# mengcaopku/DCNet

Measured on AMD Instinct MI355X. Metric: clips/sec (T=8, 416x416, bs8) fwd+bwd, higher is better.
Workload: dtype f32; 1 GPU; T=8 416x416 bs8/GPU L=20 fp32, 64 img/GPU/step as pairs, fwd+5 losses+bwd+RMSprop; arith=f16x2-split MFMA, fp32 accumulate, parallelism=dp1, ranks_seen=1, reducer=none, step=hipGraph replay (fwd+losses+bwd+RMSprop), sampler=mt

## Files before the change

dcnet_amd/csrc/conv3x.hip:

```cpp
#include "igemm.h"
#include "prof.h"
#include <type_traits>

namespace {

typedef _Float16 f16x8_t __attribute__((ext_vector_type(8)));
typedef _Float16 f16x4_t __attribute__((ext_vector_type(4)));
constexpr unsigned OOBX = 0x80000000u;

constexpr int XBM = 256, XBN = 128, XNT = 512, XWM = 4;
constexpr int XPB = XBN * 32;
constexpr int XPB1 = XPB + 64;
constexpr int XSLOT = 2 * XPB + 128;
constexpr int XSTAGE = 6 * XSLOT;
constexpr int XA_LD = 4;
#ifndef C3X_ABL
#define C3X_ABL 0
#endif
constexpr int XSMAX = 466;
constexpr int XPA = (XSMAX + 2) * 32;

__device__ __forceinline__ f32x4 ldx16(__amdgpu_buffer_rsrc_t r, unsigned voff, unsigned soff) {
  return __builtin_bit_cast(f32x4, __builtin_amdgcn_raw_buffer_load_b128(r, voff, soff, 0));
}
__device__ __forceinline__ __amdgpu_buffer_rsrc_t rsrcx(const float* base, long long bytes) {
  const unsigned n = bytes > 0x7FFFFFF0LL ? 0x7FFFFFF0u : (bytes < 0 ? 0u : (unsigned)bytes);
  return __builtin_amdgcn_make_buffer_rsrc((void*)base, 0, n, 0x00020000);
}
__device__ __forceinline__ float pow2_scalex(unsigned amax_bits) {
  const int be = (int)((amax_bits >> 23) & 0xFF);
  if (be == 0 || be == 255) return 1.f;
  int e = 14 - (be - 126);
  e = e > 100 ? 100 : (e < -100 ? -100 : e);
  return __uint_as_float((unsigned)(e + 127) << 23);
}

typedef __attribute__((address_space(3))) void lds_voidx;
template <bool DMA>
__global__ __launch_bounds__(XNT, 2) void conv3x_kernel(const IgemmParams p, const int S, const int gran) {
  extern __shared__ __attribute__((aligned(16))) unsigned char smemx[];
  constexpr int PA = XPA;
  unsigned char* const Abase = smemx;
  unsigned char* const Bbase = smemx + 4 * PA;

  const int tid = threadIdx.x, lane = tid & 63, wave = tid >> 6;
  const int wm = wave >> 1, wn = wave & 1;
  const int c16 = lane & 15, g = lane >> 4, tsel = g >> 1, half = g & 1;
  const int gn = (p.Co + XBN - 1) / XBN;
  const int lin = xcd_remap(blockIdx.x, gridDim.x);
  const int bm = lin / gn, bn = lin - bm * gn;
  const int W = p.Wi, H = p.Hi, M = p.M;
  const int m0 = bm * XBM;
  const float sa = pow2_scalex(amax_read(p.amax_a)), sb = p.b_scale[0];

  const int lin0 = m0 - W - 1;
  const int base_px = lin0 > 0 ? lin0 : 0;
  const float* a_base = p.in + (long long)base_px * p.ldi;
  const __amdgpu_buffer_rsrc_t a_rs = rsrcx(a_base, ((long long)(M - base_px - 1) * p.ldi + p.Ci) * 4);
  const __amdgpu_buffer_rsrc_t b_rs = rsrcx(p.wt, (long long)p.Co * p.ldw * 4);

  const int pos0 = tid >> 2, q0 = tid & 3;
  const unsigned a_off0 = (unsigned)((lin0 + pos0 - base_px) * p.ldi * 4 + q0 * 16);
  const int a_st0 = pos0 * 32 + q0 * 8;
  const unsigned a_pstride = (unsigned)(128 * p.ldi * 4);
  bool a_ok[XA_LD], a_in[XA_LD];
#pragma unroll
  for (int j = 0; j < XA_LD; ++j) {
    const int pos = pos0 + 128 * j, px = lin0 + pos;
    a_in[j] = pos < S;
    a_ok[j] = pos < S && px >= 0 && px < M;
  }
  auto a_off = [&](const int j) {
    unsigned o = a_off0;
    asm volatile("" : "+v"(o));
    return a_ok[j] ? o + (unsigned)j * a_pstride : OOBX;
  };
  auto a_st = [&](const int j) {
    int o = a_st0;
    asm volatile("" : "+v"(o));
    return a_in[j] ? o + j * 4096 : (XSMAX + 1) * 32 + q0 * 8;
  };
  unsigned b_off; int b_st;
  if constexpr (DMA) {
    const int plane = wave & 1, rho = 32 * (wave >> 1) + (lane >> 1), kh = lane & 1;
    const int filt = (rho & ~63) + 4 * (rho & 15) + ((rho & 63) >> 4);
    const int co = bn * XBN + filt;
    b_off = co < p.Co ? (unsigned)(co * p.ldw * 4 + (2 * kh + plane) * 16) : OOBX;
    b_st = __builtin_amdgcn_readfirstlane(plane * XPB1 + (wave >> 1) * 1024);
  } else {
    const int rho = tid >> 2, chunk = tid & 3;
    const int filt = (rho & ~63) + 4 * (rho & 15) + ((rho & 63) >> 4);
    const int co = bn * XBN + filt;
    b_off = co < p.Co ? (unsigned)(co * p.ldw * 4 + chunk * 16) : OOBX;
    b_st = (chunk & 1) * XPB1 + rho * 32 + (chunk >> 1) * 16;
  }
  unsigned msk[4];
#pragma unroll
  for (int i = 0; i < 4; ++i) {
    const int m = m0 + wm * 64 + i * 16 + c16;
    unsigned v = 0;
    if (m < M) {
      const int rem = m % (H * W), y = rem / W, x = rem - y * W;
      for (int t = 0; t < 9; ++t)
        if ((unsigned)(y + p.tap_dy[t]) < (unsigned)H && (unsigned)(x + p.tap_dx[t]) < (unsigned)W) v |= 1u << t;
    }
    msk[i] = v;
  }
  const int a_lane0 = (wm * 64 + c16) * 32 + half * 16;
  const int b_lane0 = (wn * 64 + c16) * 32 + half * 16 + tsel * 3 * XSLOT;

  const int nch = p.Ci >> 4;
  const int nper = nch >> 1;
  const int nsi = 3 * nper;

  f32x4 a_reg[XA_LD], b_reg[6];
  const unsigned lds0 = (unsigned)(uintptr_t)(lds_voidx*)smemx;
  auto store_a_piece = [&](const int buf_off, int j) {
    const f32x4 t = a_reg[j] * sa;
    const f16x4_t h = {(_Float16)t[0], (_Float16)t[1], (_Float16)t[2], (_Float16)t[3]};
    const f16x4_t l = {(_Float16)(t[0] - (float)h[0]), (_Float16)(t[1] - (float)h[1]), (_Float16)(t[2] - (float)h[2]),
                       (_Float16)(t[3] - (float)h[3])};
    if constexpr (DMA) {
      const unsigned addr = lds0 + (unsigned)(buf_off + a_st(j));
      asm volatile("ds_write_b64 %0, %1\n\tds_write_b64 %0, %2 offset:%3"
                   :: "v"(addr), "v"(__builtin_bit_cast(unsigned long long, h)), "v"(__builtin_bit_cast(unsigned long long, l)), "n"(XPA));
    } else {
      unsigned char* abuf = Abase + buf_off;
      *reinterpret_cast<uint2*>(abuf + a_st(j)) = __builtin_bit_cast(uint2, h);
      *reinterpret_cast<uint2*>(abuf + PA + a_st(j)) = __builtin_bit_cast(uint2, l);
    }
  };

  f32x4 acc[4][4];
#pragma unroll
  for (int i = 0; i < 4; ++i)
#pragma unroll
    for (int j = 0; j < 4; ++j) acc[i][j] = f32x4{0.f, 0.f, 0.f, 0.f};

  if (tid < 8) {
    const f32x4 z = {0.f, 0.f, 0.f, 0.f};
    *reinterpret_cast<f32x4*>(Abase + (tid >> 1) * PA + XSMAX * 32 + (tid & 1) * 16) = z;
  }
#pragma unroll
  for (int j = 0; j < XA_LD; ++j) a_reg[j] = ldx16(a_rs, a_off(j), 0u);
  auto dma = [&](const int stage_off, const int slot, const bool live, const unsigned soff) {
    __builtin_amdgcn_raw_ptr_buffer_load_lds(b_rs, (lds_voidx*)(Bbase + stage_off + slot * XSLOT + b_st), 16, (int)(live ? b_off : OOBX),
                                             (int)(live ? soff : 0u), 0, 0);
  };
  if constexpr (DMA) {
#pragma unroll
    for (int q = 0; q < 6; ++q) {
      const int G = q / 3, j = q - 3 * G;
      dma(0, q, true, (unsigned)p.tap_w[3 * G + j] * 4u);
    }
#pragma unroll
    for (int q = 0; q < 2; ++q)
      dma(XSTAGE, q, true, (unsigned)p.tap_w[6 + q] * 4u);
#pragma unroll
    for (int j = 0; j < XA_LD; ++j) store_a_piece(0, j);
#pragma unroll
    for (int j = 0; j < XA_LD; ++j) a_reg[j] = ldx16(a_rs, a_off(j), 64u);
    asm volatile("s_waitcnt vmcnt(0)" ::: "memory");
  } else {
#pragma unroll
    for (int q = 0; q < 6; ++q) {
      const int G = q / 3, j = q - 3 * G;
      b_reg[q] = ldx16(b_rs, b_off, (unsigned)p.tap_w[3 * G + j] * 4u);
    }
#pragma unroll
    for (int j = 0; j < XA_LD; ++j) store_a_piece(0, j);
#pragma unroll
    for (int j = 0; j < XA_LD; ++j) a_reg[j] = ldx16(a_rs, a_off(j), 64u);
#pragma unroll
    for (int q = 0; q < 6; ++q) *reinterpret_cast<f32x4*>(Bbase + q * XSLOT + b_st) = b_reg[q];
#pragma unroll
    for (int q = 0; q < 6; ++q) {
      const int G = q < 3 ? 2 : 0, cc = q < 3 ? 0 : 1, j = q % 3;
      b_reg[q] = ldx16(b_rs, b_off, (unsigned)(p.tap_w[3 * G + j] + cc * 16) * 4u);
    }
  }
  __syncthreads();

  f16x8_t Al[4], Ah[4], Bh[4], Bl[4];
  int ad[4];
  auto a_addr = [&](const int T, const int J) {
    const int Ga = T == 0 ? 0 : (T == 1 ? 2 : 1), Gb = T == 0 ? 1 : (T == 1 ? 0 : 2);
    const int ta = 3 * Ga + J, tb = 3 * Gb + J;
    const int sha = (p.tap_dy[ta] + 1) * W + p.tap_dx[ta] + 1, shb = (p.tap_dy[tb] + 1) * W + p.tap_dx[tb] + 1;
    int ts = tsel;
    asm volatile("" : "+v"(ts));
    const int sh = ts ? shb : sha;
    const int tl = ts ? tb : ta;
    const int bo = T == 0 ? 0 : (T == 2 ? 2 * PA : ts * (2 * PA));
    const int base = bo + a_lane0 + sh * 32;
    const int z = bo + XSMAX * 32;
#pragma unroll
    for (int i = 0; i < 4; ++i) ad[i] = ((msk[i] >> tl) & 1) ? base + i * 512 : z;
  };
  auto read_Al = [&]() {
#pragma unroll
    for (int i = 0; i < 4; ++i) Al[i] = *reinterpret_cast<const f16x8_t*>(Abase + PA + ad[i]);
  };
  auto read_Ah = [&]() {
#pragma unroll
    for (int i = 0; i < 4; ++i) Ah[i] = *reinterpret_cast<const f16x8_t*>(Abase + ad[i]);
  };
  int st_cur = 0;
  auto read_B = [&](f16x8_t (&B)[4], const int stage_off, const int J, const int plane) {
    const unsigned char* bb = Bbase + stage_off + b_lane0;
#pragma unroll
    for (int jn = 0; jn < 4; ++jn) B[jn] = *reinterpret_cast<const f16x8_t*>(bb + J * XSLOT + plane * XPB1 + jn * 512);
  };
  auto mm = [&](const f16x8_t (&A)[4], const f16x8_t (&B)[4]) {
#pragma unroll
    for (int i = 0; i < 4; ++i)
#pragma unroll
      for (int jn = 0; jn < 4; ++jn) acc[i][jn] = __builtin_amdgcn_mfma_f32_16x16x32_f16(A[i], B[jn], acc[i][jn], 0, 0, 0);
  };

  auto body = [&](auto T_, const int u) {
    constexpr int T = decltype(T_)::value;
    constexpr int TN = (T + 1) % 3;
    const int k = 3 * u + T, c0 = 2 * u;
    const bool in_b = k + 2 < nsi;
    const int st_nxt = XSTAGE - st_cur;
    unsigned char* const bw = Bbase + st_nxt + b_st;
    auto side = [&](const int gi) {
      if constexpr (DMA) {
        if (gi < 4 && !(C3X_ABL & 1)) {
          const int sl = gi + 2, second = sl >= 3, j = sl - 3 * second;
          const int G = T == 0 ? (second ? 0 : 2) : (T == 1 ? (second ? 2 : 1) : (second ? 1 : 0));
          const int dc = T == 0 ? (second ? 1 : 0) : (T == 1 ? 1 : 2);
          dma(st_nxt, sl, k + 1 < nsi, (unsigned)(p.tap_w[3 * G + j] + (c0 + dc) * 16) * 4u);
        }
        if (gi >= 7 && !(C3X_ABL & 1)) {
          const int sl = gi - 7;
          const int G = T == 0 ? 1 : (T == 1 ? 0 : 2), dc = T == 0 ? 1 : 2;
          dma(st_cur, sl, in_b, (unsigned)(p.tap_w[3 * G + sl] + (c0 + dc) * 16) * 4u);
        }
      } else {
      if (gi < 6 && !(C3X_ABL & 4)) *reinterpret_cast<f32x4*>(bw + gi * XSLOT) = b_reg[gi];
      if (gi >= 3 && !(C3X_ABL & 1)) {
        const int q = gi - 3, second = q >= 3, j = q - 3 * second;
        const int G = T == 0 ? (second ? 2 : 1) : (T == 1 ? (second ? 1 : 0) : (second ? 0 : 2));
        const int dc = T == 0 ? 1 : (T == 1 ? 2 : (second ? 3 : 2));
        const unsigned soff = (unsigned)(p.tap_w[3 * G + j] + (c0 + dc) * 16) * 4u;
        b_reg[q] = ldx16(b_rs, in_b ? b_off : OOBX, in_b ? soff : 0u);
      }
      }
      if (T == 0 && gi >= 2 && gi < 2 + XA_LD && !(C3X_ABL & 4)) store_a_piece(2 * PA, gi - 2);
      if (T == 1 && gi < XA_LD && !(C3X_ABL & 2)) {
        const bool in_a = c0 + 2 < nch;
        a_reg[gi] = ldx16(a_rs, in_a ? a_off(gi) : OOBX, in_a ? (unsigned)(c0 + 2) * 64u : 0u);
      }
      if (T == 2 && gi < XA_LD && !(C3X_ABL & 4)) store_a_piece(0, gi);
      if (T == 2 && gi >= 4 && gi < 4 + XA_LD && !(C3X_ABL & 2)) {
        const bool in_a = c0 + 3 < nch;
        a_reg[gi - 4] = ldx16(a_rs, in_a ? a_off(gi - 4) : OOBX, in_a ? (unsigned)(c0 + 3) * 64u : 0u);
      }
    };
#pragma unroll
    for (int j = 0; j < 3; ++j) {
      read_Ah();
      read_B(Bl, st_cur, j, 1);
      __builtin_amdgcn_sched_barrier(0);
      mm(Al, Bh);
      side(3 * j);
      __builtin_amdgcn_sched_barrier(0);
      if (j == 2 && !(C3X_ABL & 8)) {
        if constexpr (DMA) {
          if (T == 2 && !(C3X_ABL & 2)) asm volatile("s_waitcnt vmcnt(3) lgkmcnt(0)\n\ts_barrier" ::: "memory");
          else asm volatile("s_waitcnt vmcnt(0) lgkmcnt(0)\n\ts_barrier" ::: "memory");
        } else {
          __syncthreads();
        }
      }
      if (j < 2) a_addr(T, j + 1); else a_addr(TN, 0);
      read_Al();
      __builtin_amdgcn_sched_barrier(0);
      mm(Ah, Bh);
      side(3 * j + 1);
      __builtin_amdgcn_sched_barrier(0);
      if (j < 2) read_B(Bh, st_cur, j + 1, 0); else read_B(Bh, st_nxt, 0, 0);
      __builtin_amdgcn_sched_barrier(0);
      mm(Ah, Bl);
      side(3 * j + 2);
      __builtin_amdgcn_sched_barrier(0);
    }
    st_cur = st_nxt;
  };
  a_addr(0, 0);
  read_Al();
  read_B(Bh, 0, 0, 0);
  {
    using I0 = std::integral_constant<int, 0>; using I1 = std::integral_constant<int, 1>; using I2 = std::integral_constant<int, 2>;
    for (int u = 0; u < nper; ++u) { body(I0{}, u); body(I1{}, u); body(I2{}, u); }
  }
  if constexpr (DMA) asm volatile("s_waitcnt vmcnt(0)" ::: "memory");
  __syncthreads();

  const float dq = 1.f / (sa * sb);
#pragma unroll
  for (int i = 0; i < 4; ++i)
#pragma unroll
    for (int jn = 0; jn < 4; ++jn) acc[i][jn] *= dq;
  const int co0 = bn * XBN + wn * 64 + 4 * c16;
  const bool co_ok = co0 < p.Co;
  const int mrow0 = m0 + wm * 64 + 4 * g;
  float* __restrict__ gout = p.out;
  if (p.accumulate && co_ok) {
#pragma unroll
    for (int i = 0; i < 4; ++i)
#pragma unroll
      for (int r = 0; r < 4; ++r) {
        const int m = mrow0 + 16 * i + r;
        if (m >= M) continue;
        const f32x4 o = *reinterpret_cast<const f32x4*>(gout + (size_t)m * p.ldo + co0);
#pragma unroll
        for (int jn = 0; jn < 4; ++jn) acc[i][jn][r] += o[jn];
      }
  }
  if (p.stats) {
    float* red = reinterpret_cast<float*>(smemx);
    float s[4] = {0.f, 0.f, 0.f, 0.f}, ss[4] = {0.f, 0.f, 0.f, 0.f};
    if (p.bt_y && co_ok) {
      const f32x4 mu = *reinterpret_cast<const f32x4*>(p.bt_mean + co0), is = *reinterpret_cast<const f32x4*>(p.bt_invstd + co0);
      f32x4 ga = {1.f, 1.f, 1.f, 1.f}, be = {0.f, 0.f, 0.f, 0.f};
      if (p.bt_gamma) ga = *reinterpret_cast<const f32x4*>(p.bt_gamma + co0);
      if (p.bt_beta) be = *reinterpret_cast<const f32x4*>(p.bt_beta + co0);
      const float* yb = p.bt_y + co0;
#pragma unroll
      for (int i = 0; i < 4; ++i) {
        f32x4 yv[4];
#pragma unroll
        for (int r = 0; r < 4; ++r) {
          const int m = mrow0 + 16 * i + r;
          yv[r] = *reinterpret_cast<const f32x4*>(yb + (size_t)(m < M ? m : M - 1) * p.Co);
        }
#pragma unroll
        for (int r = 0; r < 4; ++r) {
          const int m = mrow0 + 16 * i + r;
#pragma unroll
          for (int jn = 0; jn < 4; ++jn) {
            const float xh = (yv[r][jn] - mu[jn]) * is[jn];
            float gq = acc[i][jn][r];
            if (p.bt_act == DCN_ACT_LEAKY) gq = (ga[jn] * xh + be[jn] <= 0.f) ? gq * p.bt_slope : gq;
            gq = m < M ? gq : 0.f;
            s[jn] += gq; ss[jn] += gq * xh;
          }
        }
      }
    } else if (!p.bt_y) {
#pragma unroll
      for (int i = 0; i < 4; ++i)
#pragma unroll
        for (int r = 0; r < 4; ++r)
#pragma unroll
          for (int jn = 0; jn < 4; ++jn) { const float v = acc[i][jn][r]; s[jn] += v; ss[jn] = __builtin_fmaf(v, v, ss[jn]); }
    }
#pragma unroll
    for (int jn = 0; jn < 4; ++jn) {
      s[jn] += __shfl_xor(s[jn], 16); ss[jn] += __shfl_xor(ss[jn], 16);
      s[jn] += __shfl_xor(s[jn], 32); ss[jn] += __shfl_xor(ss[jn], 32);
    }
    if (g == 0) {
      const int col = wn * 64 + 4 * c16;
      *reinterpret_cast<f32x4*>(red + (0 * XWM + wm) * XBN + col) = f32x4{s[0], s[1], s[2], s[3]};
      *reinterpret_cast<f32x4*>(red + (1 * XWM + wm) * XBN + col) = f32x4{ss[0], ss[1], ss[2], ss[3]};
    }
    __syncthreads();
    const int groups = XBM / gran, spg = XWM / groups;
    const int rows_total = (M + gran - 1) / gran;
    for (int idx = tid; idx < 2 * XBN * groups; idx += XNT) {
      const int gq = idx / (2 * XBN), rest = idx - gq * 2 * XBN;
      const int which = rest / XBN, col = rest - which * XBN;
      float t = 0.f;
      for (int w = 0; w < spg; ++w) t += red[(which * XWM + gq * spg + w) * XBN + col];
      const int co = bn * XBN + col, srow = bm * groups + gq;
      if (co < p.Co && srow < rows_total) p.stats[((size_t)srow * 2 + which) * p.Co + co] = t;
    }
  }
  float vmax = 0.f;
  if (co_ok) {
    f32x4 sc = {1.f, 1.f, 1.f, 1.f}, sh = {0.f, 0.f, 0.f, 0.f};
    if (p.scale) sc = *reinterpret_cast<const f32x4*>(p.scale + co0);
    if (p.shift) sh = *reinterpret_cast<const f32x4*>(p.shift + co0);
#pragma unroll
    for (int i = 0; i < 4; ++i)
#pragma unroll
      for (int r = 0; r < 4; ++r) {
        const int m = mrow0 + 16 * i + r;
        if (m >= M) continue;
        f32x4 v;
#pragma unroll
        for (int jn = 0; jn < 4; ++jn) {
          float t = acc[i][jn][r] * sc[jn] + sh[jn];
          if (p.act == DCN_ACT_LEAKY) t = t > 0.f ? t : t * p.slope;
          v[jn] = t;
        }
        if (p.residual) v += *reinterpret_cast<const f32x4*>(p.residual + (size_t)m * p.ldr + co0);
        *reinterpret_cast<f32x4*>(gout + (size_t)m * p.ldo + co0) = v;
#pragma unroll
        for (int jn = 0; jn < 4; ++jn) vmax = fmaxf(vmax, fabsf(v[jn]));
      }
  }
  if (p.amax_out) {
    vmax = wave_max(vmax);
    if (lane == 0) amax_update(p.amax_out, vmax, blockIdx.x * 8 + wave);
  }
}

}

bool conv3x_takes(const IgemmParams& p, int gran) {
  if (p.wt16 || (gran != 128 && gran != 256)) return false;
  if (p.Co % 4 != 0 || p.ldo % 4 != 0 || (p.residual && p.ldr % 4 != 0)) return false;
  auto al16 = [](const void* q) { return (reinterpret_cast<uintptr_t>(q) & 15) == 0; };
  if (!al16(p.out) || !al16(p.residual) || !al16(p.bt_y) || !al16(p.scale) || !al16(p.shift) || !al16(p.bt_mean) || !al16(p.bt_invstd) ||
      !al16(p.bt_gamma) || !al16(p.bt_beta)) return false;
  const int S = XBM + 2 * p.Wi + 2;
  if (S > XSMAX) return false;
  return (long long)S * p.ldi * 4 < 0x7FFFFFF0LL && (long long)p.Co * p.ldw * 4 < 0x7FFFFFF0LL;
}

int conv3x_launch(const IgemmParams& p, int gran, hipStream_t stream) {
  const int S = XBM + 2 * p.Wi + 2;
  const size_t lds = (size_t)4 * XPA + (size_t)2 * XSTAGE;
  static_assert((size_t)4 * XPA + (size_t)2 * XSTAGE <= 160 * 1024, "LDS");
  static DcnPerDeviceFlag attr_once;
  if (attr_once.first()) {
    (void)hipFuncSetAttribute(reinterpret_cast<const void*>(&conv3x_kernel<true>), hipFuncAttributeMaxDynamicSharedMemorySize, 160 * 1024);
  }
  const int gm = cdiv(p.M, XBM), gn = cdiv(p.Co, XBN);
  const double k_alg = 9.0 * p.Ci;
  const double alg_bytes = 4.0 * ((double)p.N * p.Hi * p.Wi * p.Ci + (double)p.Co * k_alg + (double)p.M * p.Co * epilogue_reads(p));
  const int pid = prof_begin(51, 2.0 * (double)p.M * p.Co * k_alg, stream, alg_bytes);
  hipLaunchKernelGGL(conv3x_kernel<true>, dim3(gm * gn), dim3(XNT), lds, stream, p, S, gran);
  prof_end(pid, stream);
  DCN_CHECK_LAUNCH("conv3x");
  return DCN_OK;
}
```

Measured before the change: 90.50 clips/s.

## Make conv3x persistent with next-tile prefetch overlapping the epilogue

```diff
diff --git a/dcnet_amd/csrc/conv3x.hip b/dcnet_amd/csrc/conv3x.hip
--- a/dcnet_amd/csrc/conv3x.hip
+++ b/dcnet_amd/csrc/conv3x.hip
@@ -19,6 +19,10 @@
 #endif
 constexpr int XSMAX = 466;
 constexpr int XPA = (XSMAX + 2) * 32;
+constexpr int XRED = 4 * XPA + 2 * XSTAGE;
+#ifndef C3X_WALK
+#define C3X_WALK 1
+#endif
 
 __device__ __forceinline__ f32x4 ldx16(__amdgpu_buffer_rsrc_t r, unsigned voff, unsigned soff) {
   return __builtin_bit_cast(f32x4, __builtin_amdgcn_raw_buffer_load_b128(r, voff, soff, 0));
@@ -47,29 +51,21 @@
   const int wm = wave >> 1, wn = wave & 1;
   const int c16 = lane & 15, g = lane >> 4, tsel = g >> 1, half = g & 1;
   const int gn = (p.Co + XBN - 1) / XBN;
-  const int lin = xcd_remap(blockIdx.x, gridDim.x);
-  const int bm = lin / gn, bn = lin - bm * gn;
   const int W = p.Wi, H = p.Hi, M = p.M;
-  const int m0 = bm * XBM;
+  const int tiles = ((M + XBM - 1) / XBM) * gn;
   const float sa = pow2_scalex(amax_read(p.amax_a)), sb = p.b_scale[0];
-
-  const int lin0 = m0 - W - 1;
-  const int base_px = lin0 > 0 ? lin0 : 0;
-  const float* a_base = p.in + (long long)base_px * p.ldi;
-  const __amdgpu_buffer_rsrc_t a_rs = rsrcx(a_base, ((long long)(M - base_px - 1) * p.ldi + p.Ci) * 4);
   const __amdgpu_buffer_rsrc_t b_rs = rsrcx(p.wt, (long long)p.Co * p.ldw * 4);
 
+  int bm, bn, m0;
+  __amdgpu_buffer_rsrc_t a_rs;
+
   const int pos0 = tid >> 2, q0 = tid & 3;
-  const unsigned a_off0 = (unsigned)((lin0 + pos0 - base_px) * p.ldi * 4 + q0 * 16);
+  unsigned a_off0;
   const int a_st0 = pos0 * 32 + q0 * 8;
   const unsigned a_pstride = (unsigned)(128 * p.ldi * 4);
   bool a_ok[XA_LD], a_in[XA_LD];
 #pragma unroll
-  for (int j = 0; j < XA_LD; ++j) {
-    const int pos = pos0 + 128 * j, px = lin0 + pos;
-    a_in[j] = pos < S;
-    a_ok[j] = pos < S && px >= 0 && px < M;
-  }
+  for (int j = 0; j < XA_LD; ++j) a_in[j] = pos0 + 128 * j < S;
   auto a_off = [&](const int j) {
     unsigned o = a_off0;
     asm volatile("" : "+v"(o));
@@ -80,32 +76,45 @@
     asm volatile("" : "+v"(o));
     return a_in[j] ? o + j * 4096 : (XSMAX + 1) * 32 + q0 * 8;
   };
-  unsigned b_off; int b_st;
+  unsigned b_off; int b_st, b_filt, b_chunk;
   if constexpr (DMA) {
     const int plane = wave & 1, rho = 32 * (wave >> 1) + (lane >> 1), kh = lane & 1;
-    const int filt = (rho & ~63) + 4 * (rho & 15) + ((rho & 63) >> 4);
-    const int co = bn * XBN + filt;
-    b_off = co < p.Co ? (unsigned)(co * p.ldw * 4 + (2 * kh + plane) * 16) : OOBX;
+    b_filt = (rho & ~63) + 4 * (rho & 15) + ((rho & 63) >> 4);
+    b_chunk = 2 * kh + plane;
     b_st = __builtin_amdgcn_readfirstlane(plane * XPB1 + (wave >> 1) * 1024);
   } else {
     const int rho = tid >> 2, chunk = tid & 3;
-    const int filt = (rho & ~63) + 4 * (rho & 15) + ((rho & 63) >> 4);
-    const int co = bn * XBN + filt;
-    b_off = co < p.Co ? (unsigned)(co * p.ldw * 4 + chunk * 16) : OOBX;
+    b_filt = (rho & ~63) + 4 * (rho & 15) + ((rho & 63) >> 4);
+    b_chunk = chunk;
     b_st = (chunk & 1) * XPB1 + rho * 32 + (chunk >> 1) * 16;
   }
   unsigned msk[4];
-#pragma unroll
-  for (int i = 0; i < 4; ++i) {
-    const int m = m0 + wm * 64 + i * 16 + c16;
-    unsigned v = 0;
-    if (m < M) {
-      const int rem = m % (H * W), y = rem / W, x = rem - y * W;
-      for (int t = 0; t < 9; ++t)
-        if ((unsigned)(y + p.tap_dy[t]) < (unsigned)H && (unsigned)(x + p.tap_dx[t]) < (unsigned)W) v |= 1u << t;
-    }
-    msk[i] = v;
-  }
+  auto tile_setup = [&](const int t) {
+    const int lin = xcd_remap(t, tiles);
+    bm = lin / gn; bn = lin - bm * gn; m0 = bm * XBM;
+    const int lin0 = m0 - W - 1;
+    const int base_px = lin0 > 0 ? lin0 : 0;
+    a_rs = rsrcx(p.in + (long long)base_px * p.ldi, ((long long)(M - base_px - 1) * p.ldi + p.Ci) * 4);
+    a_off0 = (unsigned)((lin0 + pos0 - base_px) * p.ldi * 4 + q0 * 16);
+#pragma unroll
+    for (int j = 0; j < XA_LD; ++j) {
+      const int px = lin0 + pos0 + 128 * j;
+      a_ok[j] = a_in[j] && px >= 0 && px < M;
+    }
+    const int co = bn * XBN + b_filt;
+    b_off = co < p.Co ? (unsigned)(co * p.ldw * 4 + b_chunk * 16) : OOBX;
+#pragma unroll
+    for (int i = 0; i < 4; ++i) {
+      const int m = m0 + wm * 64 + i * 16 + c16;
+      unsigned v = 0;
+      if (m < M) {
+        const int rem = m % (H * W), y = rem / W, x = rem - y * W;
+        for (int t9 = 0; t9 < 9; ++t9)
+          if ((unsigned)(y + p.tap_dy[t9]) < (unsigned)H && (unsigned)(x + p.tap_dx[t9]) < (unsigned)W) v |= 1u << t9;
+      }
+      msk[i] = v;
+    }
+  };
   const int a_lane0 = (wm * 64 + c16) * 32 + half * 16;
   const int b_lane0 = (wn * 64 + c16) * 32 + half * 16 + tsel * 3 * XSLOT;
 
@@ -132,54 +141,56 @@
   };
 
   f32x4 acc[4][4];
-#pragma unroll
-  for (int i = 0; i < 4; ++i)
-#pragma unroll
-    for (int j = 0; j < 4; ++j) acc[i][j] = f32x4{0.f, 0.f, 0.f, 0.f};
 
   if (tid < 8) {
     const f32x4 z = {0.f, 0.f, 0.f, 0.f};
     *reinterpret_cast<f32x4*>(Abase + (tid >> 1) * PA + XSMAX * 32 + (tid & 1) * 16) = z;
   }
-#pragma unroll
-  for (int j = 0; j < XA_LD; ++j) a_reg[j] = ldx16(a_rs, a_off(j), 0u);
   auto dma = [&](const int stage_off, const int slot, const bool live, const unsigned soff) {
     __builtin_amdgcn_raw_ptr_buffer_load_lds(b_rs, (lds_voidx*)(Bbase + stage_off + slot * XSLOT + b_st), 16, (int)(live ? b_off : OOBX),
                                              (int)(live ? soff : 0u), 0, 0);
   };
-  if constexpr (DMA) {
-#pragma unroll
-    for (int q = 0; q < 6; ++q) {
-      const int G = q / 3, j = q - 3 * G;
-      dma(0, q, true, (unsigned)p.tap_w[3 * G + j] * 4u);
-    }
-#pragma unroll
-    for (int q = 0; q < 2; ++q)
-      dma(XSTAGE, q, true, (unsigned)p.tap_w[6 + q] * 4u);
-#pragma unroll
-    for (int j = 0; j < XA_LD; ++j) store_a_piece(0, j);
-#pragma unroll
-    for (int j = 0; j < XA_LD; ++j) a_reg[j] = ldx16(a_rs, a_off(j), 64u);
-    asm volatile("s_waitcnt vmcnt(0)" ::: "memory");
-  } else {
-#pragma unroll
-    for (int q = 0; q < 6; ++q) {
-      const int G = q / 3, j = q - 3 * G;
-      b_reg[q] = ldx16(b_rs, b_off, (unsigned)p.tap_w[3 * G + j] * 4u);
-    }
-#pragma unroll
-    for (int j = 0; j < XA_LD; ++j) store_a_piece(0, j);
-#pragma unroll
-    for (int j = 0; j < XA_LD; ++j) a_reg[j] = ldx16(a_rs, a_off(j), 64u);
-#pragma unroll
-    for (int q = 0; q < 6; ++q) *reinterpret_cast<f32x4*>(Bbase + q * XSLOT + b_st) = b_reg[q];
-#pragma unroll
-    for (int q = 0; q < 6; ++q) {
-      const int G = q < 3 ? 2 : 0, cc = q < 3 ? 0 : 1, j = q % 3;
-      b_reg[q] = ldx16(b_rs, b_off, (unsigned)(p.tap_w[3 * G + j] + cc * 16) * 4u);
-    }
-  }
-  __syncthreads();
+  auto tile_first_loads = [&]() {
+#pragma unroll
+    for (int j = 0; j < XA_LD; ++j) a_reg[j] = ldx16(a_rs, a_off(j), 0u);
+    if constexpr (DMA) {
+#pragma unroll
+      for (int q = 0; q < 6; ++q) {
+        const int G = q / 3, j = q - 3 * G;
+        dma(0, q, true, (unsigned)p.tap_w[3 * G + j] * 4u);
+      }
+#pragma unroll
+      for (int q = 0; q < 2; ++q)
+        dma(XSTAGE, q, true, (unsigned)p.tap_w[6 + q] * 4u);
+    }
+  };
+  auto tile_prologue = [&]() {
+    if constexpr (DMA) {
+#pragma unroll
+      for (int j = 0; j < XA_LD; ++j) store_a_piece(0, j);
+#pragma unroll
+      for (int j = 0; j < XA_LD; ++j) a_reg[j] = ldx16(a_rs, a_off(j), 64u);
+      asm volatile("s_waitcnt vmcnt(0)" ::: "memory");
+    } else {
+#pragma unroll
+      for (int q = 0; q < 6; ++q) {
+        const int G = q / 3, j = q - 3 * G;
+        b_reg[q] = ldx16(b_rs, b_off, (unsigned)p.tap_w[3 * G + j] * 4u);
+      }
+#pragma unroll
+      for (int j = 0; j < XA_LD; ++j) store_a_piece(0, j);
+#pragma unroll
+      for (int j = 0; j < XA_LD; ++j) a_reg[j] = ldx16(a_rs, a_off(j), 64u);
+#pragma unroll
+      for (int q = 0; q < 6; ++q) *reinterpret_cast<f32x4*>(Bbase + q * XSLOT + b_st) = b_reg[q];
+#pragma unroll
+      for (int q = 0; q < 6; ++q) {
+        const int G = q < 3 ? 2 : 0, cc = q < 3 ? 0 : 1, j = q % 3;
+        b_reg[q] = ldx16(b_rs, b_off, (unsigned)(p.tap_w[3 * G + j] + cc * 16) * 4u);
+      }
+    }
+    __syncthreads();
+  };
 
   f16x8_t Al[4], Ah[4], Bh[4], Bl[4];
   int ad[4];
@@ -289,6 +300,15 @@
     }
     st_cur = st_nxt;
   };
+  tile_setup(blockIdx.x);
+  tile_first_loads();
+  for (int tile = blockIdx.x;;) {
+#pragma unroll
+  for (int i = 0; i < 4; ++i)
+#pragma unroll
+    for (int j = 0; j < 4; ++j) acc[i][j] = f32x4{0.f, 0.f, 0.f, 0.f};
+  tile_prologue();
+  st_cur = 0;
   a_addr(0, 0);
   read_Al();
   read_B(Bh, 0, 0, 0);
@@ -299,14 +319,19 @@
   if constexpr (DMA) asm volatile("s_waitcnt vmcnt(0)" ::: "memory");
   __syncthreads();
 
+  const int bm_e = bm, bn_e = bn, m0_e = m0;
+  tile += gridDim.x;
+  const bool more = tile < tiles;
+  if (more) { tile_setup(tile); tile_first_loads(); }
+
   const float dq = 1.f / (sa * sb);
 #pragma unroll
   for (int i = 0; i < 4; ++i)
 #pragma unroll
     for (int jn = 0; jn < 4; ++jn) acc[i][jn] *= dq;
-  const int co0 = bn * XBN + wn * 64 + 4 * c16;
+  const int co0 = bn_e * XBN + wn * 64 + 4 * c16;
   const bool co_ok = co0 < p.Co;
-  const int mrow0 = m0 + wm * 64 + 4 * g;
+  const int mrow0 = m0_e + wm * 64 + 4 * g;
   float* __restrict__ gout = p.out;
   if (p.accumulate && co_ok) {
 #pragma unroll
@@ -321,7 +346,7 @@
       }
   }
   if (p.stats) {
-    float* red = reinterpret_cast<float*>(smemx);
+    float* red = reinterpret_cast<float*>(smemx + XRED);
     float s[4] = {0.f, 0.f, 0.f, 0.f}, ss[4] = {0.f, 0.f, 0.f, 0.f};
     if (p.bt_y && co_ok) {
       const f32x4 mu = *reinterpret_cast<const f32x4*>(p.bt_mean + co0), is = *reinterpret_cast<const f32x4*>(p.bt_invstd + co0);
@@ -376,7 +401,7 @@
       const int which = rest / XBN, col = rest - which * XBN;
       float t = 0.f;
       for (int w = 0; w < spg; ++w) t += red[(which * XWM + gq * spg + w) * XBN + col];
-      const int co = bn * XBN + col, srow = bm * groups + gq;
+      const int co = bn_e * XBN + col, srow = bm_e * groups + gq;
       if (co < p.Co && srow < rows_total) p.stats[((size_t)srow * 2 + which) * p.Co + co] = t;
     }
   }
@@ -407,6 +432,8 @@
   if (p.amax_out) {
     vmax = wave_max(vmax);
     if (lane == 0) amax_update(p.amax_out, vmax, blockIdx.x * 8 + wave);
+  }
+  if (!more) break;
   }
 }
 
@@ -425,17 +452,19 @@
 
 int conv3x_launch(const IgemmParams& p, int gran, hipStream_t stream) {
   const int S = XBM + 2 * p.Wi + 2;
-  const size_t lds = (size_t)4 * XPA + (size_t)2 * XSTAGE;
-  static_assert((size_t)4 * XPA + (size_t)2 * XSTAGE <= 160 * 1024, "LDS");
+  const size_t lds = (size_t)XRED + sizeof(float) * 2 * XWM * XBN;
+  static_assert((size_t)XRED + sizeof(float) * 2 * XWM * XBN <= 160 * 1024 && XRED % 16 == 0, "LDS");
   static DcnPerDeviceFlag attr_once;
   if (attr_once.first()) {
     (void)hipFuncSetAttribute(reinterpret_cast<const void*>(&conv3x_kernel<true>), hipFuncAttributeMaxDynamicSharedMemorySize, 160 * 1024);
   }
   const int gm = cdiv(p.M, XBM), gn = cdiv(p.Co, XBN);
+  const int tiles = gm * gn, cus = dcn_device_cus();
+  const int grid = C3X_WALK && cus > 0 && cus % 8 == 0 && tiles > cus ? cus : tiles;
   const double k_alg = 9.0 * p.Ci;
   const double alg_bytes = 4.0 * ((double)p.N * p.Hi * p.Wi * p.Ci + (double)p.Co * k_alg + (double)p.M * p.Co * epilogue_reads(p));
   const int pid = prof_begin(51, 2.0 * (double)p.M * p.Co * k_alg, stream, alg_bytes);
-  hipLaunchKernelGGL(conv3x_kernel<true>, dim3(gm * gn), dim3(XNT), lds, stream, p, S, gran);
+  hipLaunchKernelGGL(conv3x_kernel<true>, dim3(grid), dim3(XNT), lds, stream, p, S, gran);
   prof_end(pid, stream);
   DCN_CHECK_LAUNCH("conv3x");
   return DCN_OK;
```

Result: no change. 90.95 clips/s (median of 6 runs) (+0.5%).
